# deepalcoholic/mlcomp

Measured on AMD Instinct MI355X. Metric: images/sec (whole node) ResNet-50 DAG train task, higher is better.
Workload: dtype bf16; 1 GPU; model=resnet50, global_batch=512, per_gpu_batch=512, image_size=224, parallelism=dp1, impl=native, optimizer=SGD momentum 0.9, wd 5e-5, fp32 master weights

## Files before the change

csrc/kernels/igemm.hip:

```cpp
#include "gfx950.h"
#include "convgeom.h"
#include <stdlib.h>
#include <map>
#include <mutex>
#include <vector>
#include <algorithm>
#include <cstdio>

namespace igemm {

constexpr int BK = 64, NTHR = 256;


template <int R>
__device__ __forceinline__ int mc_off(int k, int c) {
  if (R == 64) return k * 128 + ((c ^ (((k >> 1) & 1) << 2)) << 4);
  return k * (R * 2) + ((c ^ ((k & 3) << 2)) << 4);
}

template <class L, int R>
__device__ __forceinline__ void store_stage(char* lds, int tid, const uint4 (&v)[R / 32]) {
#pragma unroll
  for (int i = 0; i < R / 32; ++i) *reinterpret_cast<uint4*>(lds + L::lds_off(i, tid)) = v[i];
}
// ... 472 lines not shown
      ldg8f(bn.sc + st.ci[c], a);
      ldg8f(bn.sh + st.ci[c], b);
#pragma unroll
      for (int j = 0; j < 2; ++j) {
        const bool ok = (unsigned)(hb[j] + st.rd[c]) < (unsigned)g.H && (unsigned)(wb[j] + st.sd[c]) < (unsigned)g.W;
        v[2 * c + j] = bn_relu8(v[2 * c + j], a, b, ok);
      }
    }
  }
};


struct IdentityRows {
  __device__ __forceinline__ size_t operator()(int m) const { return (size_t)m; }
};
struct ClassRows {
  DgradClass c; int H, W;
  __device__ __forceinline__ size_t operator()(int m) const {
    int n, i, j;
    c.decode(m, n, i, j);
    return ((size_t)n * H + i * c.S + c.ph) * W + j * c.S + c.pw;
  }
};

struct BnBwdEpi {
  const bf16* mask = nullptr;
  const bf16* y0 = nullptr; const float* mean0 = nullptr; float* sums0 = nullptr;
  const bf16* y1 = nullptr; const float* mean1 = nullptr; float* sums1 = nullptr;
  const float* msc0 = nullptr; const float* msh0 = nullptr;
  const float* msc1 = nullptr; const float* msh1 = nullptr;
  int ncopy = NSTAT;
};

__device__ __forceinline__ float erf_from_exp(float x, float e) {
  const float t = __builtin_amdgcn_rcpf(1.f + 0.3275911f * fabsf(x));
  const float p = ((((1.061405429f * t - 1.453152027f) * t + 1.421413741f) * t - 0.284496736f) * t + 0.254829592f) * t;
  return copysignf(1.f - p * e, x);
}

__device__ __forceinline__ void dense_act8(float (&a)[8], int act, bf16* pre) {
  const int mode = act & 3;
  if (mode == 3) {
    if (pre) *reinterpret_cast<uint4*>(pre) = pack8(a);
#pragma unroll
    for (int e = 0; e < 8; ++e) a[e] = fmaxf(a[e], 0.f);
    return;
// ... 105 lines not shown
      if (aff) { ldg8f(bn.msc0 + ncl, ma0); ldg8f(bn.msh0 + ncl, mb0); }
      if (aff1) { ldg8f(bn.msc1 + ncl, ma1); ldg8f(bn.msh1 + ncl, mb1); }
    }
    const bool dense = kDense && (bias || act || dact);
    float bz[8];
#pragma unroll
    for (int e = 0; e < 8; ++e) bz[e] = 0.f;
    if (kDense && bias) ldg8f(bias + (nc < N ? nc : 0), bz);
    constexpr int ITERS = (BM + RPI - 1) / RPI;
    if (!addend && !red && !dense) {
#pragma unroll
      for (int it = 0; it < ITERS; ++it) {
        const int row = tid / CPR + RPI * it;
        const int m = m0 + row;
        if ((EXACT || (tok && row < BM)) && m < M && nc < N)
          *reinterpret_cast<uint4*>(out + rowmap(m) * ld + nc) =
              *reinterpret_cast<const uint4*>(lds + row * RS + c * 16);
      }
      return;
    }
    constexpr int UMAX = kDense ? 4 : 8;
    constexpr int U = ITERS < UMAX ? ITERS : UMAX;
    const bool has_add = addend != nullptr, has_mask = red && bn.mask, has_y1 = red && bn.y1;
#pragma unroll 1
    for (int it0 = 0; it0 < ITERS; it0 += U) {
      constexpr int UB = kDense ? 1 : U;
      constexpr int UD = kDense ? U : 1;
      uint4 vv[U], aa[U], zz[UB], p0[UB], p1[UB], du[UD];
      size_t off[U];
      bool ok[U];
#pragma unroll
      for (int u = 0; u < U; ++u) {
        int row = tid / CPR + RPI * (it0 + u);
        const bool rin = EXACT || (tok && row < BM);
        if (!rin) row = 0;
        const int m = m0 + row;
        ok[u] = rin && m < M && nc < N;
        off[u] = ok[u] ? rowmap(m) * ld + nc : 0;
        vv[u] = *reinterpret_cast<const uint4*>(lds + row * RS + c * 16);
        const uint4 zero = make_uint4(0u, 0u, 0u, 0u);
        aa[u] = has_add ? ldg16(addend + off[u]) : zero;
        if constexpr (!kDense) {
          zz[u] = has_mask ? ldg16(bn.mask + off[u]) : zero;
          p0[u] = red ? ldg16(bn.y0 + off[u]) : zero;
          p1[u] = has_y1 ? ldg16(bn.y1 + off[u]) : zero;
        }
        if constexpr (kDense) du[u] = dact ? ldg16(dact + off[u]) : zero;
      }
#pragma unroll
      for (int u = 0; u < U; ++u) {
        if (!ok[u]) continue;
        uint4 v = vv[u];
        if (has_add || red || dense) {
          float a[8];
          unpack8(v, a);
          if constexpr (kDense) {
          if (bias) {
#pragma unroll
            for (int e = 0; e < 8; ++e) a[e] += bz[e];
          }
          dense_act8(a, act, preact ? preact + off[u] : nullptr);
          if (dact) dense_dact8(a, act, du[u]);
          }
          if (has_add) {
            float b[8];
            unpack8(aa[u], b);
#pragma unroll
            for (int e = 0; e < 8; ++e) a[e] += b[e];
          }
          if constexpr (!kDense) {
            if (has_mask) {
              float z[8];
              unpack8(zz[u], z);
#pragma unroll
              for (int e = 0; e < 8; ++e) a[e] = z[e] > 0.f ? a[e] : 0.f;
            } else if (aff) {
              float y[8], q[8];
              unpack8(p0[u], y);
#pragma unroll
              for (int e = 0; e < 8; ++e) q[e] = y[e] * ma0[e] + mb0[e];
              if (aff1) {
                unpack8(p1[u], y);
#pragma unroll
                for (int e = 0; e < 8; ++e) q[e] += y[e] * ma1[e] + mb1[e];
              }
#pragma unroll
              for (int e = 0; e < 8; ++e) a[e] = q[e] > 0.f ? a[e] : 0.f;
// ... 897 lines not shown
  const MkMatKC fb{w, K, Co, K};
  if (KH == 1 && KW == 1 && stride == 1 && pad == 0) {
    if (in_sc) return launch_tiles(tile, M, Co, K, 1, st, epi, MkMatKCBn{x, C, M, K, bn}, fb);
    return launch_tiles(tile, M, Co, K, 1, st, epi, MkMatKC{x, C, M, K}, fb);
  }
  const ConvGeom g = mkgeom(N, H, W, C, Co, KH, KW, stride, pad, dil, Ho, Wo);
  if (in_sc) return launch_tiles(tile, M, Co, K, 1, st, epi, MkConvFwdABn{x, g, M, K, bn}, fb);
  return launch_tiles(tile, M, Co, K, 1, st, epi, MkConvFwdA{x, g, M, K}, fb);
}

MLC_EXPORT int mlc_conv_fwd(const bf16* x, const bf16* w, bf16* y, float* sum, float* sumsq,
                            int N, int H, int W, int C, int Co, int KH, int KW, int stride,
                            int pad, int dil, int Ho, int Wo, const float* in_sc, const float* in_sh,
                            hipStream_t st) {
  return conv_fwd_impl(x, w, y, Co, sum, sumsq, N, H, W, C, Co, KH, KW, stride, pad, dil, Ho, Wo, in_sc, in_sh, st);
}

MLC_EXPORT int mlc_conv_fwd_ld(const bf16* x, const bf16* w, bf16* y, int ldy, int N, int H, int W, int C, int Co,
                               int KH, int KW, int stride, int pad, int dil, int Ho, int Wo, hipStream_t st) {
  return conv_fwd_impl(x, w, y, ldy, nullptr, nullptr, N, H, W, C, Co, KH, KW, stride, pad, dil, Ho, Wo, nullptr,
                       nullptr, st);
}

static int dgrad_check(const BnBwdEpi& bn, int N, int H, int W, int C, int Co, int KH, int KW, int stride,
                       const float* sum, const float* sumsq) {
  if (C % 8 || Co % 8 || KH > 15 || KW > 16 || stride < 1 || ((sum == nullptr) != (sumsq == nullptr))) return -1;
  if (bn.y0 && g_mlc_det && ((long)N * H * W + 63) / 64 > g_mlc_ncopy) return -2;
  if (bn.msc0 && (!bn.msh0 || !bn.y0 || (bn.msc1 && (!bn.msh1 || !bn.y1)))) return -1;
  if (bn.y0 && (!bn.mean0 || !bn.sums0 || (bn.y1 && (!bn.mean1 || !bn.sums1)))) return -1;
  return 0;
}

template <class MkB>
static int dgrad_classes(const bf16* dy, const bf16* w, bf16* dx, const bf16* addend, const BnBwdEpi& bn,
                         const ConvGeom& g, int pad, float* sum, float* sumsq, hipStream_t st) {
  hipError_t err = hipSuccess;
  for (int ph = 0; ph < g.stride && ph < g.H; ++ph)
    for (int pw = 0; pw < g.stride && pw < g.W; ++pw) {
      const DgradClass cl = mkclass(g.stride, ph, pw, g.H, g.W, g.Ho, g.Wo, g.Co, g.KH, g.KW, pad, g.dil);
      if (cl.nr > 15 || cl.ns > 16) return -1;
      const int M = g.N * cl.Hc * cl.Wc, K = cl.nr * cl.ns * cl.ncb * BK;
      if (M <= 0) continue;
      if (sum && g_mlc_det && (M + 63) / 64 > g_mlc_ncopy) return -2;
      const int tile = pick_tile(M, g.C);
      const MkConvDgradA fa{dy, g, M, K, cl};
      const MkB fb{w, g, cl};
      if (g.stride == 1) {
        EpiBF16<> epi{dx, g.C, sum, sumsq, IdentityRows{}, addend, bn};
        epi.ncopy = g_mlc_ncopy;
        err = launch_tiles(tile, M, g.C, K, 1, st, epi, fa, fb);
      } else {
        EpiBF16<ClassRows> epi{dx, g.C, sum, sumsq, ClassRows{cl, g.H, g.W}, addend, bn};
        epi.ncopy = g_mlc_ncopy;
        err = launch_tiles(tile, M, g.C, K, 1, st, epi, fa, fb);
      }
      if (err != hipSuccess) return err;
    }
  return err;
}

static int conv_dgrad_impl(const bf16* dy, const bf16* w, bf16* dx, const bf16* addend, int N,
                           int H, int W, int C, int Co, int KH, int KW, int stride, int pad,
                           int dil, int Ho, int Wo, const bf16* bn_mask, const bf16* bn_y0,
                           const float* bn_mean0, float* bn_sums0, const bf16* bn_y1,
                           const float* bn_mean1, float* bn_sums1, const float* bn_msc0,
                           const float* bn_msh0, const float* bn_msc1, const float* bn_msh1,
                           float* sum, float* sumsq, hipStream_t st) {
  const BnBwdEpi bn{bn_mask, bn_y0, bn_mean0, bn_sums0, bn_y1, bn_mean1, bn_sums1,
                    bn_msc0, bn_msh0, bn_msc1, bn_msh1, g_mlc_ncopy};
  if (const int rc = dgrad_check(bn, N, H, W, C, Co, KH, KW, stride, sum, sumsq)) return rc;
  const ConvGeom g = mkgeom(N, H, W, C, Co, KH, KW, stride, pad, dil, Ho, Wo);
  if (KH == 1 && KW == 1 && stride == 1 && pad == 0) {
    const DgradClass cl = mkclass(1, 0, 0, H, W, Ho, Wo, Co, 1, 1, 0, dil);
    const int M = N * H * W, K = cl.ncb * BK;
    if (sum && g_mlc_det && (M + 63) / 64 > g_mlc_ncopy) return -2;
    EpiBF16<> epi{dx, C, sum, sumsq, IdentityRows{}, addend, bn};
    epi.ncopy = g_mlc_ncopy;
    return launch_tiles(pick_tile(M, C), M, C, K, 1, st, epi, MkMatKC{dy, Co, M, Co}, MkConvDgradB{w, g, cl});
  }
  return dgrad_classes<MkConvDgradB>(dy, w, dx, addend, bn, g, pad, sum, sumsq, st);
}

MLC_EXPORT int mlc_conv_dgrad(const bf16* dy, const bf16* w, bf16* dx, const bf16* addend, int N,
                              int H, int W, int C, int Co, int KH, int KW, int stride, int pad,
                              int dil, int Ho, int Wo, const bf16* bn_mask, const bf16* bn_y0,
                              const float* bn_mean0, float* bn_sums0, const bf16* bn_y1,
                              const float* bn_mean1, float* bn_sums1, const float* bn_msc0,
                              const float* bn_msh0, const float* bn_msc1, const float* bn_msh1,
                              hipStream_t st) {
  return conv_dgrad_impl(dy, w, dx, addend, N, H, W, C, Co, KH, KW, stride, pad, dil, Ho, Wo, bn_mask, bn_y0,
                         bn_mean0, bn_sums0, bn_y1, bn_mean1, bn_sums1, bn_msc0, bn_msh0, bn_msc1, bn_msh1,
                         nullptr, nullptr, st);
}

MLC_EXPORT int mlc_conv_tr_fwd(const bf16* x, const bf16* w, bf16* y, float* sum, float* sumsq, int N, int Hi,
                               int Wi, int Cin, int Cout, int KH, int KW, int stride, int pad, int dil, int Ho,
                               int Wo, hipStream_t st) {
  int pad_h, pad_w;
  unpack_pad(pad, pad_h, pad_w);
  if (Hi != (Ho + 2 * pad_h - dil * (KH - 1) - 1) / stride + 1 || Wi != (Wo + 2 * pad_w - dil * (KW - 1) - 1) / stride + 1)
    return -1;
  return conv_dgrad_impl(x, w, y, nullptr, N, Ho, Wo, Cout, Cin, KH, KW, stride, pad, dil, Hi, Wi, nullptr,
                         nullptr, nullptr, nullptr, nullptr, nullptr, nullptr, nullptr, nullptr, nullptr,
                         nullptr, sum, sumsq, st);
}

MLC_EXPORT int mlc_conv_dgrad_t(const bf16* dy, const bf16* wt, bf16* dx, const bf16* addend, int N,
                                int H, int W, int C, int Co, int KH, int KW, int stride, int pad,
                                int dil, int Ho, int Wo, const bf16* bn_mask, const bf16* bn_y0,
                                const float* bn_mean0, float* bn_sums0, const bf16* bn_y1,
                                const float* bn_mean1, float* bn_sums1, const float* bn_msc0,
                                const float* bn_msh0, const float* bn_msc1, const float* bn_msh1,
                                hipStream_t st) {
  const BnBwdEpi bn{bn_mask, bn_y0, bn_mean0, bn_sums0, bn_y1, bn_mean1, bn_sums1,
                    bn_msc0, bn_msh0, bn_msc1, bn_msh1, g_mlc_ncopy};
  if (const int rc = dgrad_check(bn, N, H, W, C, Co, KH, KW, stride, nullptr, nullptr)) return rc;
  int pad_h, pad_w;
  unpack_pad(pad, pad_h, pad_w);
  const int ph = dil * (KH - 1) - pad_h, pw = dil * (KW - 1) - pad_w;
  if (stride == 1 && ph >= 0 && pw >= 0) {
    if (Ho != H + 2 * pad_h - dil * (KH - 1) || Wo != W + 2 * pad_w - dil * (KW - 1)) return -1;
    const int M = N * H * W, K = KH * KW * Co;
    const int tile = pick_tile(M, C);
    EpiBF16<> epi{dx, C, nullptr, nullptr, IdentityRows{}, addend, bn};
    const MkMatKC fb{wt, K, C, K};
    if (KH == 1 && KW == 1) return launch_tiles(tile, M, C, K, 1, st, epi, MkMatKC{dy, Co, M, Co}, fb);
    const ConvGeom gf = mkgeom(N, Ho, Wo, Co, C, KH, KW, 1, pack_pad(ph, pw), dil, H, W);
    return launch_tiles(tile, M, C, K, 1, st, epi, MkConvFwdA{dy, gf, M, K}, fb);
  }
  const ConvGeom g = mkgeom(N, H, W, C, Co, KH, KW, stride, pad, dil, Ho, Wo);
  return dgrad_classes<MkConvDgradBT>(dy, wt, dx, addend, bn, g, pad, nullptr, nullptr, st);
}

namespace {
__global__ void __launch_bounds__(256)
splitk_reduce_kernel(const float* __restrict__ ws, float* __restrict__ out, long n4, int splits,
                     long slab4, int accumulate) {
  typedef float v4 __attribute__((ext_vector_type(4)));
  const v4* w4 = reinterpret_cast<const v4*>(ws);
  v4* o4 = reinterpret_cast<v4*>(out);
  for (long i = (long)blockIdx.x * 256 + threadIdx.x; i < n4; i += (long)gridDim.x * 256) {
    v4 a = accumulate ? o4[i] : (v4){0.f, 0.f, 0.f, 0.f};
    v4 b = {0.f, 0.f, 0.f, 0.f};
    int k = 0;
    for (; k + 4 <= splits; k += 4) {
      const v4 u0 = w4[(k + 0) * slab4 + i], u1 = w4[(k + 1) * slab4 + i];
      const v4 u2 = w4[(k + 2) * slab4 + i], u3 = w4[(k + 3) * slab4 + i];
      a += u0 + u1;
      b += u2 + u3;
    }
    for (; k < splits; ++k) a += w4[k * slab4 + i];
    o4[i] = a + b;
  }
}
// ... 237 lines not shown
```

mlcomp_amd/ops/_lib.py:

```python
from __future__ import annotations

import ctypes as C
import os
import threading

import torch

_LIB = None
_LOCK = threading.Lock()

DETERMINISTIC = os.environ.get('MLC_DETERMINISTIC', '0') == '1'
DET_COPIES = max(32, int(os.environ.get('MLC_DET_COPIES', '4096')))

vp, i32, i64, f32, u32 = C.c_void_p, C.c_int, C.c_long, C.c_float, C.c_uint

_SIGS = {
    'mlc_conv_fwd': [vp, vp, vp, vp, vp] + [i32] * 12 + [vp, vp, vp],
    'mlc_conv_fwd_ld': [vp, vp, vp] + [i32] * 13 + [vp],
    'mlc_conv_dgrad': [vp] * 4 + [i32] * 12 + [vp] * 11 + [vp],
    'mlc_conv_dgrad_t': [vp] * 4 + [i32] * 12 + [vp] * 11 + [vp],
    'mlc_bilinear_up_fwd': [vp, vp] + [i32] * 6 + [vp],
    'mlc_bilinear_up_bwd': [vp, vp] + [i32] * 6 + [vp],
    'mlc_gn_relu_fwd': [vp, vp, vp, vp, vp] + [i32] * 4 + [f32, vp],
    'mlc_gn_relu_bwd': [vp] * 7 + [i32] * 4 + [f32, vp],
    'mlc_conv_tr_fwd': [vp] * 5 + [i32] * 12 + [vp],
    'mlc_wt_transpose': [vp, i32, i64, vp],
    'mlc_conv_wgrad': [vp, vp, vp] + [i32] * 14 + [vp, i64, vp, vp, vp],
    'mlc_conv_wgrad_native': [vp, vp, vp] + [i32] * 14 + [vp, i64, vp, vp, vp],
    'mlc_gemm_f32out': [vp, vp, vp, vp] + [i32] * 11 + [vp],
    'mlc_gemm_bf16out': [vp, vp, vp] + [i32] * 8 + [vp],
    'mlc_gemm256_nt': [vp, vp, vp, vp] + [i32] * 6 + [vp, i32, vp, vp, i32, i32, vp],
    'mlc_g256_dense': [vp, vp, vp] + [i32] * 7 + [vp, i32, vp, vp, vp, i32, vp],
    'mlc_gemm256_tn': [vp, vp, vp] + [i32] * 8 + [vp],
    'mlc_conv256_fwd': [vp] * 5 + [i32] * 13 + [vp],
    'mlc_augment': [vp, vp, vp, vp] + [i32] * 7 + [vp],
    'mlc_augment_seg': [vp] * 6 + [i32] * 9 + [vp],
    'mlc_gemm_bf16_ex': [vp, vp, vp] + [i32] * 8 + [vp, i32, vp, vp, vp, vp, i64, vp],
    'mlc_gemm_bf16_ex_native': [vp, vp, vp] + [i32] * 8 + [vp, i32, vp, vp, vp, vp, i64, vp],
    'mlc_ln_fwd': [vp] * 8 + [i32, i32, f32, f32, f32, vp, u32, u32, vp],
    'mlc_ln_bwd': [vp] * 10 + [i32, i32, f32, f32, vp, u32, u32, vp],
    'mlc_ln_finalize_many': [vp, i32, i32, vp],
    'mlc_embed_bwd': [vp] * 7 + [i32] * 4 + [vp],
    'mlc_softmax_fwd': [vp] * 4 + [i64, i32, i32, f32, f32, vp, u32, vp],
# ... 175 lines not shown
```

mlcomp_amd/ops/functional.py:

```python
from __future__ import annotations

from typing import Optional, Tuple

import contextlib
import math
import os
import threading

import torch
import torch.nn.functional as F

from . import _lib


def _cuda(t):
    return t is not None and t.is_cuda


def conv_out_hw(H, W, KH, KW, stride, pad, dil):
    ph, pw = (pad, pad) if isinstance(pad, int) else tuple(pad)
    Ho = (H + 2 * ph - dil * (KH - 1) - 1) // stride + 1
    Wo = (W + 2 * pw - dil * (KW - 1) - 1) // stride + 1
    return Ho, Wo

# ... 191 lines not shown
        rows, blk = [], 0
        for s, v in zip(self.slots, self.views):
            Co, KH, KW, Ci = self._dims(s.shape)
            rows.append([s.bf16.data_ptr(), v.data_ptr(), Co, KH * KW, Ci, blk])
            blk += KH * KW * ((Co + 63) // 64) * ((Ci + 63) // 64)
        self.desc = torch.tensor(rows, dtype=torch.int64).to(self.buf.device)
        self.blocks = blk
        self._srcs = [r[0] for r in rows]

    def refresh(self):
        if self.buf is None:
            return
        if not self.buf.is_cuda:
            for s, v in zip(self.slots, self.views):
                v.copy_(wt_flip_transpose(s.bf16) if s.bf16.dim() == 4 else s.bf16.t())
            return
        if self._srcs != [s.bf16.data_ptr() for s in self.slots]:
            self._build()
        _lib.call('mlc_wt_transpose', _lib.ptr(self.desc), len(self.slots), self.blocks, _lib.stream())


def conv2d_dgrad(dy: torch.Tensor, w: torch.Tensor, x_shape, stride=1, pad=0, dil=1,
                 addend: Optional[torch.Tensor] = None, out: Optional[torch.Tensor] = None,
                 bn: Optional[BnBwdSpec] = None, wt: Optional[torch.Tensor] = None) -> torch.Tensor:
    N, H, W, C = x_shape
    Co, KH, KW, Ci = w.shape
    _, Ho, Wo, _ = dy.shape
    if _cuda(dy):
        dx = out if out is not None else torch.empty(N, H, W, C, device=dy.device, dtype=torch.bfloat16)
        b = [None] * 11
        if bn is not None:
            b[0] = bn.mask
            for k, (yk, mk, sk) in enumerate(bn.ys):
                b[1 + 3 * k:4 + 3 * k] = [yk, mk, sk]
            for k, (ak, hk) in enumerate(bn.affine or []):
                b[7 + 2 * k:9 + 2 * k] = [ak, hk]
        if wt is not None:
            assert tuple(wt.shape) == (Ci, KH, KW, Co), (wt.shape, w.shape)
            _lib.call('mlc_conv_dgrad_t', _lib.ptr(dy), _lib.ptr(wt), _lib.ptr(dx), _lib.ptr(addend), N, H, W,
                      C, Co, KH, KW, stride, pack_pad(pad), dil, Ho, Wo, *[_lib.ptr(t) for t in b], _lib.stream())
            return dx
        _lib.call('mlc_conv_dgrad', _lib.ptr(dy), _lib.ptr(w), _lib.ptr(dx), _lib.ptr(addend), N, H, W, C,
                  Co, KH, KW, stride, pack_pad(pad), dil, Ho, Wo, *[_lib.ptr(t) for t in b], _lib.stream())
        return dx
    if wt is not None and isinstance(pad, int) and dgrad_as_fwd_conv(KH, KW, stride, pad, dil):
        dxf = F.conv2d(dy.permute(0, 3, 1, 2).float(), wt.permute(0, 3, 1, 2).float(), None, 1,
                       dil * (KH - 1) - pad, dil)
    else:
        if wt is not None:
            w = wt_flip_transpose(wt)
        dxf = torch.nn.grad.conv2d_input((N, C, H, W), w.permute(0, 3, 1, 2).float(),
                                         dy.permute(0, 3, 1, 2).float(), stride, pad, dil)
    dxf = dxf.permute(0, 2, 3, 1)
    if addend is not None:
        dxf = dxf + addend.float()
    if bn is not None:
        if bn.mask is not None:
            dxf = dxf * (bn.mask.float() > 0)
        elif bn.affine is not None:
            q = sum(yk.float() * ak + hk for (yk, _, _), (ak, hk) in zip(bn.ys, bn.affine))
            dxf = dxf * (q > 0)
        d = dxf.to(torch.bfloat16).float().reshape(-1, C)
        for yk, mk, sk in bn.ys:
            sv = sk.view(NSTAT, 2, C)
            sv[0, 0] += d.sum(0)
            sv[0, 1] += (d * (yk.float().reshape(-1, C) - mk)).sum(0)
    dx = dxf.to(torch.bfloat16).contiguous()
    if out is not None:
        out.copy_(dx)
        return out
    return dx


_USE_SLAB = os.environ.get('MLC_WGRAD_SLAB', '1') != '0'
_SLAB = {}
_SLAB_OLD = []


# ... 1200 lines not shown
```

mlcomp_amd/ops/layers.py:

```python
from __future__ import annotations

import math
import os
from typing import List, Optional

import torch
import torch.nn as nn

from . import functional as Fn
from .arena import ParamArena, Slot

DGRAD_FIRST_ENV = os.environ.get('MLC_DGRAD_FIRST')


class Workspace:

    def __init__(self):
        self._req: List[tuple] = []
        self.buf = None
        self.views = {}

    def request(self, key, n):
        self._req.append((key, int(n)))
        return key

    def finalize(self, device):
        total = sum((n + 63) // 64 * 64 for _, n in self._req) or 64
        self.buf = torch.zeros(total, device=device, dtype=torch.float32)
        off = 0
        for key, n in self._req:
            self.views[key] = self.buf[off:off + n]
            off += (n + 63) // 64 * 64

    def __getitem__(self, key):
        return self.views[key]
# ... 221 lines not shown
        if self.s2d and in_affine is None:
            return Fn.stem_conv_fwd(x, self.w.bf16, stats=stats)
        if stats is not None and in_affine is None and self._conv1x1_fwd_ok(x):
            return Fn.conv1x1_fwd(x, self.w.bf16, stats)
        return Fn.conv2d_fwd(x, self.w.bf16, self.stride, self.pad, self.dil, stats=stats, in_affine=in_affine)

    def _conv1x1_fwd_ok(self, x) -> bool:
        if not (Fn.CONV1X1_FWD and x.is_cuda and type(self) is ConvBN and not self.s2d):
            return False
        if self.k != (1, 1) or self.stride != 1 or self.pad != 0 or x.shape[-1] != self.cin_p:
            return False
        return Fn.conv1x1_fwd_available(self.cin_p, self.Co)

    def _conv1x1_res_ok(self, x) -> bool:
        if not (Fn.CONV1X1_RES and x.is_cuda and type(self) is ConvBN and not self.s2d):
            return False
        if self.k != (1, 1) or self.stride != 1 or self.pad != 0 or x.shape[-1] != self.cin_p:
            return False
        min_rows = Fn.conv1x1_res_min_rows(self.cin_p, self.Co)
        if min_rows is None or math.prod(x.shape[:-1]) < min_rows:
            return False
        return Fn.conv1x1_fwd_res_available(self.cin_p, self.Co)

    def _dgrad(self, dy, x_shape, addend=None, out=None, bn=None):
        wt = None
        if self.wt_idx is not None:
            if self.ctx.wt_stale:
                raise RuntimeError('transposed filters are stale: the model must call '
                                   'ctx.refresh_wt() after its training forward pass')
            wt = self.ctx.wt[self.wt_idx]
        return Fn.conv2d_dgrad(dy, self.w.bf16, x_shape, self.stride, self.pad, self.dil,
                               addend=addend, out=out, bn=bn, wt=wt)

    def dgrad_covers_all(self) -> bool:
        return True

    def bn_target(self, rec):
        x, y, z = rec
        return (y, self.save_mean, self.ctx.ws[self.k_bw])

    def wgrad(self, dy, x, in_affine=None):
        Fn.conv2d_wgrad(dy, x, self.w.shape, self.stride, self.pad, self.dil, out=self.w.grad,
                        accumulate=self.ctx.grad_prezeroed, in_affine=in_affine, slab=self.ctx.wgrad_slab)
        if self.s2d:
            self.w.grad.mul_(self._gmask)

    def _fused_1x1_bwd_ok(self, dz, x, dgrad_bn) -> bool:
        if not (Fn.FUSE_1X1_BWD and dz.is_cuda and type(self) is ConvBN and not self.s2d):
            return False
        if self.k != (1, 1) or self.stride != 1 or self.pad != 0 or x.shape[-1] != self.cin_p:
            return False
        if dgrad_bn is not None and (dgrad_bn.mask is not None or len(dgrad_bn.ys) != 1
                                     or dgrad_bn.affine is None):
            return False
        return Fn.conv1x1_bn_bwd_available(self.cin_p, self.Co)

    def bwd(self, dz, rec, want_dres=False, dx_addend=None, need_dx=True, dx_out=None,
            prereduced=False, dgrad_bn=None, in_affine=None, defer: Optional[list] = None):
        x, y, z = rec
        arena = self.ctx.arena
        if need_dx and prereduced and in_affine is None and self._fused_1x1_bwd_ok(dz, x, dgrad_bn):
            if not self.ctx.grad_prezeroed:
                self.w.grad.zero_()
            dx = Fn.conv1x1_bn_bwd(dz, y, x, self.w.bf16, self.save_mean, self.save_invstd,
                                   self.gamma.master, self.ctx.ws[self.k_bw], self.gamma.grad,
                                   self.beta.grad, self.w.grad, addend=dx_addend, out=dx_out, bn=dgrad_bn)
            arena.mark_ready(self.gamma)
            arena.mark_ready(self.beta)
            arena.mark_ready(self.w)
            return dx, (dz if want_dres else None)
        dy, dres = Fn.bn_bwd(dz, z if self.act else None, y, self.save_mean, self.save_invstd,
                             self.gamma.master, want_dres=want_dres, dgamma=self.gamma.grad,
                             dbeta=self.beta.grad, sums=self.ctx.ws[self.k_bw], zero_sums=False,
                             coef=self.coef, prereduced=prereduced)
        arena.mark_ready(self.gamma)
        arena.mark_ready(self.beta)
        side = self.ctx.wgrad_stream if need_dx else None
        if side is not None and torch.cuda.current_stream(self.ctx.device) == side:
            side = None
        fork = None
        if side is not None:
            main = torch.cuda.current_stream(self.ctx.device)
            fork = torch.cuda.Event()
            fork.record(main)
            if not self.ctx.dgrad_first:
                side.wait_event(fork)
                with Fn.side_stream(side):
                    self.wgrad(dy, x, in_affine)
        else:
            self.wgrad(dy, x, in_affine)
        dx = None
        if need_dx:
            dx = self._dgrad(dy, x.shape, addend=dx_addend, out=dx_out, bn=dgrad_bn)
        if side is not None and self.ctx.dgrad_first:
            side.wait_event(fork)
            with Fn.side_stream(side):
                self.wgrad(dy, x, in_affine)
        if side is not None and defer is not None:
            defer.append((dy, x, self.w))
            return dx, dres
        if side is not None and self.ctx.wgrad_defer:
            dy.record_stream(side)
            x.record_stream(side)
            arena.mark_ready(self.w)
            return dx, dres
        if side is not None and self.ctx.wgrad_lag:
            ev = torch.cuda.Event()
            ev.record(side)
            self.ctx.lag_wgrad(ev, (dy, x), self.w)
            return dx, dres
        if side is not None:
            main.wait_stream(side)
        arena.mark_ready(self.w)
        return dx, dres


# ... 31 lines not shown
    def load_from_torch(self):
        super().load_from_torch()
        b = self._bias()
        if b is not None:
            self.run_mean.sub_(b)

    def export_to_torch(self):
        super().export_to_torch()
        b = self._bias()
        if b is not None:
            bn = self._src[1]
            bn.running_mean.add_(b.to(bn.running_mean.device))

    def out_hw(self, H, W):
        KH, KW = self.k
        return ((H - 1) * self.stride - 2 * self.pad + self.dil * (KH - 1) + self.out_pad[0] + 1,
                (W - 1) * self.stride - 2 * self.pad + self.dil * (KW - 1) + self.out_pad[1] + 1)

    def _conv(self, x, stats, in_affine=None):
        assert in_affine is None
        return Fn.conv_transpose2d_fwd(x, self.w.bf16, self.out_hw(x.shape[1], x.shape[2]), self.stride,
                                       self.pad, self.dil, stats=stats)

    def _dgrad(self, dy, x_shape, addend=None, out=None, bn=None):
        assert addend is None and out is None and bn is None, 'ConvTBN input gradient: plain conv'
        dx = Fn.conv2d_fwd(dy, self.w.bf16, self.stride, self.pad, self.dil)
        assert tuple(dx.shape) == tuple(x_shape), (dx.shape, x_shape)
        return dx

    def wgrad(self, dy, x, in_affine=None):
        assert in_affine is None
        Fn.conv2d_wgrad(x, dy, self.w.shape, self.stride, self.pad, self.dil, out=self.w.grad,
                        accumulate=self.ctx.grad_prezeroed)


class _ConvBNFn(torch.autograd.Function):
    @staticmethod
    def forward(ctx, x, res, anchor, m: ConvBN):
        z, rec = m.fwd(x, res)
        ctx.m = m
        ctx.has_res = res is not None
        ctx.save_for_backward(*rec)
        return z

    @staticmethod
    def backward(ctx, dz):
        m: ConvBN = ctx.m
        dx, dres = m.bwd(dz.contiguous(), ctx.saved_tensors, want_dres=ctx.has_res,
# ... 105 lines not shown
        blk.dout_prereduced = False
        units = blk.units
        fuse = blk.fuse_bn_bwd
        affs = blk.in_affines()
        if blk.fuse_bn_fwd:
            assert fuse, 'the BN-apply fusion needs the fused BN-backward reductions (z is not stored)'

        def spec_for(i):
            u = units[i]
            if not fuse or not units[i + 1].dgrad_covers_all():
                return None
            if u.act:
                return Fn.BnBwdSpec(None, [u.bn_target(recs[i])], affine=[(u.scale, u.shift)])
            return Fn.BnBwdSpec(None, [u.bn_target(recs[i])])

        side = units[0].ctx.wgrad_stream
        pend = [] if side is not None and os.environ.get('MLC_WGRAD_STREAM') == '2' else None
        sp = spec_for(len(units) - 2) if len(units) > 1 else None
        d, dres = units[-1].bwd(dout, recs[-1], want_dres=True, prereduced=pre, dgrad_bn=sp,
                                in_affine=affs[-1], defer=pend)
        fused = sp is not None
        down_side = side if (blk.down is not None and pend is None and blk.down_stream) else None
        short = dres
        if down_side is not None:
            main = torch.cuda.current_stream(units[0].ctx.device)
            short_buf = torch.empty(rd[0].shape, device=rd[0].device, dtype=rd[0].dtype) if need_dx else None
            down_side.wait_stream(main)
            with Fn.side_stream(down_side):
                short, _ = blk.down.bwd(dres, rd, need_dx=need_dx, prereduced=pre, dx_out=short_buf)
        for i in range(len(units) - 2, 0, -1):
            sp = spec_for(i - 1)
            d, _ = units[i].bwd(d, recs[i], prereduced=fused, dgrad_bn=sp, in_affine=affs[i], defer=pend)
            fused = sp is not None
        if down_side is not None:
            main.wait_stream(down_side)
        elif blk.down is not None:
            short, _ = blk.down.bwd(dres, rd, need_dx=need_dx, prereduced=pre, defer=pend)
        prev_spec = None
        if need_dx and fuse and blk.prev is not None and blk.prev._last is not None \
                and units[0].dgrad_covers_all():
            prev_spec = blk.prev.output_bn_spec()
        dx, _ = units[0].bwd(d, recs[0], dx_addend=short if need_dx else None, need_dx=need_dx,
                             dx_out=short if (need_dx and blk.down is not None) else None,
                             prereduced=fused, dgrad_bn=prev_spec, defer=pend)
        if prev_spec is not None:
            blk.prev.dout_prereduced = True
        if pend:
            torch.cuda.current_stream(units[0].ctx.device).wait_stream(side)
            for _, _, w in pend:
                units[0].ctx.arena.mark_ready(w)
            pend.clear()
        return dx, None, None


class MaxPool:
    def __init__(self, k=3, s=2, p=1):
        self.k, self.s, self.p = k, s, p

    def __call__(self, x, anchor):
        return _MaxPoolFn.apply(x, anchor, self)


class _MaxPoolFn(torch.autograd.Function):
    @staticmethod
    def forward(ctx, x, anchor, m):
        y, idx = Fn.maxpool_fwd(x, m.k, m.s, m.p)
        ctx.m = m
# ... 114 lines not shown
```

Before: 14420 images/s.

## Compute strided 1x1 shortcut dgrad compactly and scatter-add it in dgrad epilogue

For strided 1x1 downsample convs, the shortcut input gradient is now computed at the output resolution only, as a compact tensor, instead of a full-resolution dx that is mostly zeros. The block's first conv dgrad epilogue then adds this compact gradient at the strided positions, decoding each pixel with fast division. This removes the zero-filled work and memory traffic of the strided dgrad. In exchange it adds per-row divmod work in the epilogue, bypasses the fused 1x1 backward path whenever a strided addend is present, and allocates a new epilogue template instantiation.

Measured after the change: 14600 images/s, median of 6. +1.2%, better.

```diff
diff --git a/csrc/kernels/igemm.hip b/csrc/kernels/igemm.hip
--- a/csrc/kernels/igemm.hip
+++ b/csrc/kernels/igemm.hip
@@ -518,6 +518,22 @@
     return ((size_t)n * H + i * c.S + c.ph) * W + j * c.S + c.pw;
   }
 };
+template <class Rows = IdentityRows>
+struct StridedAddRows {
+  Rows rows; int Ho, Wo; FastDiv fW, fH, fS;
+  __device__ __forceinline__ size_t operator()(int m) const { return rows(m); }
+  __device__ __forceinline__ bool addend_pixel(size_t pix, size_t& cpix) const {
+    unsigned t, n, h, w, hq, hr, wq, wr;
+    fW.divmod((unsigned)pix, t, w);
+    fH.divmod(t, n, h);
+    fS.divmod(h, hq, hr);
+    fS.divmod(w, wq, wr);
+    cpix = ((size_t)n * Ho + hq) * Wo + wq;
+    return (hr | wr) == 0;
+  }
+};
+template <class R> struct HasStridedAdd { static constexpr bool value = false; };
+template <class R> struct HasStridedAdd<StridedAddRows<R>> { static constexpr bool value = true; };
 
 struct BnBwdEpi {
   const bf16* mask = nullptr;
@@ -669,13 +685,14 @@
     constexpr int UMAX = kDense ? 4 : 8;
     constexpr int U = ITERS < UMAX ? ITERS : UMAX;
     const bool has_add = addend != nullptr, has_mask = red && bn.mask, has_y1 = red && bn.y1;
+    constexpr bool kSAdd = HasStridedAdd<RowMap>::value;
 #pragma unroll 1
     for (int it0 = 0; it0 < ITERS; it0 += U) {
       constexpr int UB = kDense ? 1 : U;
       constexpr int UD = kDense ? U : 1;
       uint4 vv[U], aa[U], zz[UB], p0[UB], p1[UB], du[UD];
       size_t off[U];
-      bool ok[U];
+      bool ok[U], hit[U];
 #pragma unroll
       for (int u = 0; u < U; ++u) {
         int row = tid / CPR + RPI * (it0 + u);
@@ -683,10 +700,18 @@
         if (!rin) row = 0;
         const int m = m0 + row;
         ok[u] = rin && m < M && nc < N;
-        off[u] = ok[u] ? rowmap(m) * ld + nc : 0;
+        const size_t pix = ok[u] ? rowmap(m) : 0;
+        off[u] = ok[u] ? pix * ld + nc : 0;
         vv[u] = *reinterpret_cast<const uint4*>(lds + row * RS + c * 16);
         const uint4 zero = make_uint4(0u, 0u, 0u, 0u);
-        aa[u] = has_add ? ldg16(addend + off[u]) : zero;
+        if constexpr (kSAdd) {
+          size_t cpix = 0;
+          hit[u] = has_add && ok[u] && rowmap.addend_pixel(pix, cpix);
+          aa[u] = hit[u] ? ldg16(addend + cpix * ld + nc) : zero;
+        } else {
+          hit[u] = has_add;
+          aa[u] = has_add ? ldg16(addend + off[u]) : zero;
+        }
         if constexpr (!kDense) {
           zz[u] = has_mask ? ldg16(bn.mask + off[u]) : zero;
           p0[u] = red ? ldg16(bn.y0 + off[u]) : zero;
@@ -709,7 +734,7 @@
           dense_act8(a, act, preact ? preact + off[u] : nullptr);
           if (dact) dense_dact8(a, act, du[u]);
           }
-          if (has_add) {
+          if (hit[u]) {
             float b[8];
             unpack8(aa[u], b);
 #pragma unroll
@@ -1653,17 +1678,39 @@
                        nullptr, st);
 }
 
-static int dgrad_check(const BnBwdEpi& bn, int N, int H, int W, int C, int Co, int KH, int KW, int stride,
-                       const float* sum, const float* sumsq) {
+struct DgradAddend {
+  const bf16* same = nullptr; const bf16* compact = nullptr; int S = 1;
+};
+
+static int dgrad_check(const BnBwdEpi& bn, const DgradAddend& add, int N, int H, int W, int C, int Co, int KH,
+                       int KW, int stride, const float* sum, const float* sumsq) {
   if (C % 8 || Co % 8 || KH > 15 || KW > 16 || stride < 1 || ((sum == nullptr) != (sumsq == nullptr))) return -1;
+  if (add.S < 1 || (add.compact && add.same)) return -1;
   if (bn.y0 && g_mlc_det && ((long)N * H * W + 63) / 64 > g_mlc_ncopy) return -2;
   if (bn.msc0 && (!bn.msh0 || !bn.y0 || (bn.msc1 && (!bn.msh1 || !bn.y1)))) return -1;
   if (bn.y0 && (!bn.mean0 || !bn.sums0 || (bn.y1 && (!bn.mean1 || !bn.sums1)))) return -1;
   return 0;
 }
 
+template <class Rows, class FA, class FB>
+static hipError_t launch_dgrad(const Rows& rows, bf16* dx, const DgradAddend& add, const BnBwdEpi& bn, float* sum,
+                               float* sumsq, int H, int W, int M, int C, int K, hipStream_t st, const FA& fa,
+                               const FB& fb) {
+  const int tile = pick_tile(M, C);
+  if (add.compact) {
+    const StridedAddRows<Rows> srows{rows, (H - 1) / add.S + 1, (W - 1) / add.S + 1, FastDiv(W), FastDiv(H),
+                                     FastDiv(add.S)};
+    EpiBF16<StridedAddRows<Rows>> epi{dx, C, sum, sumsq, srows, add.compact, bn};
+    epi.ncopy = g_mlc_ncopy;
+    return launch_tiles(tile, M, C, K, 1, st, epi, fa, fb);
+  }
+  EpiBF16<Rows> epi{dx, C, sum, sumsq, rows, add.same, bn};
+  epi.ncopy = g_mlc_ncopy;
+  return launch_tiles(tile, M, C, K, 1, st, epi, fa, fb);
+}
+
 template <class MkB>
-static int dgrad_classes(const bf16* dy, const bf16* w, bf16* dx, const bf16* addend, const BnBwdEpi& bn,
+static int dgrad_classes(const bf16* dy, const bf16* w, bf16* dx, const DgradAddend& add, const BnBwdEpi& bn,
                          const ConvGeom& g, int pad, float* sum, float* sumsq, hipStream_t st) {
   hipError_t err = hipSuccess;
   for (int ph = 0; ph < g.stride && ph < g.H; ++ph)
@@ -1673,24 +1720,18 @@
       const int M = g.N * cl.Hc * cl.Wc, K = cl.nr * cl.ns * cl.ncb * BK;
       if (M <= 0) continue;
       if (sum && g_mlc_det && (M + 63) / 64 > g_mlc_ncopy) return -2;
-      const int tile = pick_tile(M, g.C);
       const MkConvDgradA fa{dy, g, M, K, cl};
       const MkB fb{w, g, cl};
-      if (g.stride == 1) {
-        EpiBF16<> epi{dx, g.C, sum, sumsq, IdentityRows{}, addend, bn};
-        epi.ncopy = g_mlc_ncopy;
-        err = launch_tiles(tile, M, g.C, K, 1, st, epi, fa, fb);
-      } else {
-        EpiBF16<ClassRows> epi{dx, g.C, sum, sumsq, ClassRows{cl, g.H, g.W}, addend, bn};
-        epi.ncopy = g_mlc_ncopy;
-        err = launch_tiles(tile, M, g.C, K, 1, st, epi, fa, fb);
-      }
+      if (g.stride == 1)
+        err = launch_dgrad(IdentityRows{}, dx, add, bn, sum, sumsq, g.H, g.W, M, g.C, K, st, fa, fb);
+      else
+        err = launch_dgrad(ClassRows{cl, g.H, g.W}, dx, add, bn, sum, sumsq, g.H, g.W, M, g.C, K, st, fa, fb);
       if (err != hipSuccess) return err;
     }
   return err;
 }
 
-static int conv_dgrad_impl(const bf16* dy, const bf16* w, bf16* dx, const bf16* addend, int N,
+static int conv_dgrad_impl(const bf16* dy, const bf16* w, bf16* dx, const DgradAddend& add, int N,
                            int H, int W, int C, int Co, int KH, int KW, int stride, int pad,
                            int dil, int Ho, int Wo, const bf16* bn_mask, const bf16* bn_y0,
                            const float* bn_mean0, float* bn_sums0, const bf16* bn_y1,
@@ -1699,17 +1740,16 @@
                            float* sum, float* sumsq, hipStream_t st) {
   const BnBwdEpi bn{bn_mask, bn_y0, bn_mean0, bn_sums0, bn_y1, bn_mean1, bn_sums1,
                     bn_msc0, bn_msh0, bn_msc1, bn_msh1, g_mlc_ncopy};
-  if (const int rc = dgrad_check(bn, N, H, W, C, Co, KH, KW, stride, sum, sumsq)) return rc;
+  if (const int rc = dgrad_check(bn, add, N, H, W, C, Co, KH, KW, stride, sum, sumsq)) return rc;
   const ConvGeom g = mkgeom(N, H, W, C, Co, KH, KW, stride, pad, dil, Ho, Wo);
   if (KH == 1 && KW == 1 && stride == 1 && pad == 0) {
     const DgradClass cl = mkclass(1, 0, 0, H, W, Ho, Wo, Co, 1, 1, 0, dil);
     const int M = N * H * W, K = cl.ncb * BK;
     if (sum && g_mlc_det && (M + 63) / 64 > g_mlc_ncopy) return -2;
-    EpiBF16<> epi{dx, C, sum, sumsq, IdentityRows{}, addend, bn};
-    epi.ncopy = g_mlc_ncopy;
-    return launch_tiles(pick_tile(M, C), M, C, K, 1, st, epi, MkMatKC{dy, Co, M, Co}, MkConvDgradB{w, g, cl});
-  }
-  return dgrad_classes<MkConvDgradB>(dy, w, dx, addend, bn, g, pad, sum, sumsq, st);
+    return launch_dgrad(IdentityRows{}, dx, add, bn, sum, sumsq, H, W, M, C, K, st, MkMatKC{dy, Co, M, Co},
+                        MkConvDgradB{w, g, cl});
+  }
+  return dgrad_classes<MkConvDgradB>(dy, w, dx, add, bn, g, pad, sum, sumsq, st);
 }
 
 MLC_EXPORT int mlc_conv_dgrad(const bf16* dy, const bf16* w, bf16* dx, const bf16* addend, int N,
@@ -1719,9 +1759,21 @@
                               const float* bn_mean1, float* bn_sums1, const float* bn_msc0,
                               const float* bn_msh0, const float* bn_msc1, const float* bn_msh1,
                               hipStream_t st) {
-  return conv_dgrad_impl(dy, w, dx, addend, N, H, W, C, Co, KH, KW, stride, pad, dil, Ho, Wo, bn_mask, bn_y0,
-                         bn_mean0, bn_sums0, bn_y1, bn_mean1, bn_sums1, bn_msc0, bn_msh0, bn_msc1, bn_msh1,
+  return conv_dgrad_impl(dy, w, dx, DgradAddend{addend}, N, H, W, C, Co, KH, KW, stride, pad, dil, Ho, Wo, bn_mask,
+                         bn_y0, bn_mean0, bn_sums0, bn_y1, bn_mean1, bn_sums1, bn_msc0, bn_msh0, bn_msc1, bn_msh1,
                          nullptr, nullptr, st);
+}
+
+MLC_EXPORT int mlc_conv_dgrad_sadd(const bf16* dy, const bf16* w, bf16* dx, const bf16* addend, const bf16* sadd,
+                                   int sadd_stride, int N, int H, int W, int C, int Co, int KH, int KW,
+                                   int stride, int pad, int dil, int Ho, int Wo, const bf16* bn_mask,
+                                   const bf16* bn_y0, const float* bn_mean0, float* bn_sums0, const bf16* bn_y1,
+                                   const float* bn_mean1, float* bn_sums1, const float* bn_msc0,
+                                   const float* bn_msh0, const float* bn_msc1, const float* bn_msh1,
+                                   hipStream_t st) {
+  return conv_dgrad_impl(dy, w, dx, DgradAddend{addend, sadd, sadd_stride}, N, H, W, C, Co, KH, KW, stride, pad, dil,
+                         Ho, Wo, bn_mask, bn_y0, bn_mean0, bn_sums0, bn_y1, bn_mean1, bn_sums1, bn_msc0, bn_msh0,
+                         bn_msc1, bn_msh1, nullptr, nullptr, st);
 }
 
 MLC_EXPORT int mlc_conv_tr_fwd(const bf16* x, const bf16* w, bf16* y, float* sum, float* sumsq, int N, int Hi,
@@ -1731,9 +1783,37 @@
   unpack_pad(pad, pad_h, pad_w);
   if (Hi != (Ho + 2 * pad_h - dil * (KH - 1) - 1) / stride + 1 || Wi != (Wo + 2 * pad_w - dil * (KW - 1) - 1) / stride + 1)
     return -1;
-  return conv_dgrad_impl(x, w, y, nullptr, N, Ho, Wo, Cout, Cin, KH, KW, stride, pad, dil, Hi, Wi, nullptr,
+  return conv_dgrad_impl(x, w, y, DgradAddend{}, N, Ho, Wo, Cout, Cin, KH, KW, stride, pad, dil, Hi, Wi, nullptr,
                          nullptr, nullptr, nullptr, nullptr, nullptr, nullptr, nullptr, nullptr, nullptr,
                          nullptr, sum, sumsq, st);
+}
+
+static int conv_dgrad_t_impl(const bf16* dy, const bf16* wt, bf16* dx, const DgradAddend& add, int N,
+                             int H, int W, int C, int Co, int KH, int KW, int stride, int pad,
+                             int dil, int Ho, int Wo, const bf16* bn_mask, const bf16* bn_y0,
+                             const float* bn_mean0, float* bn_sums0, const bf16* bn_y1,
+                             const float* bn_mean1, float* bn_sums1, const float* bn_msc0,
+                             const float* bn_msh0, const float* bn_msc1, const float* bn_msh1,
+                             hipStream_t st) {
+  const BnBwdEpi bn{bn_mask, bn_y0, bn_mean0, bn_sums0, bn_y1, bn_mean1, bn_sums1,
+                    bn_msc0, bn_msh0, bn_msc1, bn_msh1, g_mlc_ncopy};
+  if (const int rc = dgrad_check(bn, add, N, H, W, C, Co, KH, KW, stride, nullptr, nullptr)) return rc;
+  int pad_h, pad_w;
+  unpack_pad(pad, pad_h, pad_w);
+  const int ph = dil * (KH - 1) - pad_h, pw = dil * (KW - 1) - pad_w;
+  if (stride == 1 && ph >= 0 && pw >= 0) {
+    if (Ho != H + 2 * pad_h - dil * (KH - 1) || Wo != W + 2 * pad_w - dil * (KW - 1)) return -1;
+    const int M = N * H * W, K = KH * KW * Co;
+    const MkMatKC fb{wt, K, C, K};
+    if (KH == 1 && KW == 1)
+      return launch_dgrad(IdentityRows{}, dx, add, bn, nullptr, nullptr, H, W, M, C, K, st, MkMatKC{dy, Co, M, Co},
+                          fb);
+    const ConvGeom gf = mkgeom(N, Ho, Wo, Co, C, KH, KW, 1, pack_pad(ph, pw), dil, H, W);
+    return launch_dgrad(IdentityRows{}, dx, add, bn, nullptr, nullptr, H, W, M, C, K, st, MkConvFwdA{dy, gf, M, K},
+                        fb);
+  }
+  const ConvGeom g = mkgeom(N, H, W, C, Co, KH, KW, stride, pad, dil, Ho, Wo);
+  return dgrad_classes<MkConvDgradBT>(dy, wt, dx, add, bn, g, pad, nullptr, nullptr, st);
 }
 
 MLC_EXPORT int mlc_conv_dgrad_t(const bf16* dy, const bf16* wt, bf16* dx, const bf16* addend, int N,
@@ -1743,24 +1823,21 @@
                                 const float* bn_mean1, float* bn_sums1, const float* bn_msc0,
                                 const float* bn_msh0, const float* bn_msc1, const float* bn_msh1,
                                 hipStream_t st) {
-  const BnBwdEpi bn{bn_mask, bn_y0, bn_mean0, bn_sums0, bn_y1, bn_mean1, bn_sums1,
-                    bn_msc0, bn_msh0, bn_msc1, bn_msh1, g_mlc_ncopy};
-  if (const int rc = dgrad_check(bn, N, H, W, C, Co, KH, KW, stride, nullptr, nullptr)) return rc;
-  int pad_h, pad_w;
-  unpack_pad(pad, pad_h, pad_w);
-  const int ph = dil * (KH - 1) - pad_h, pw = dil * (KW - 1) - pad_w;
-  if (stride == 1 && ph >= 0 && pw >= 0) {
-    if (Ho != H + 2 * pad_h - dil * (KH - 1) || Wo != W + 2 * pad_w - dil * (KW - 1)) return -1;
-    const int M = N * H * W, K = KH * KW * Co;
-    const int tile = pick_tile(M, C);
-    EpiBF16<> epi{dx, C, nullptr, nullptr, IdentityRows{}, addend, bn};
-    const MkMatKC fb{wt, K, C, K};
-    if (KH == 1 && KW == 1) return launch_tiles(tile, M, C, K, 1, st, epi, MkMatKC{dy, Co, M, Co}, fb);
-    const ConvGeom gf = mkgeom(N, Ho, Wo, Co, C, KH, KW, 1, pack_pad(ph, pw), dil, H, W);
-    return launch_tiles(tile, M, C, K, 1, st, epi, MkConvFwdA{dy, gf, M, K}, fb);
-  }
-  const ConvGeom g = mkgeom(N, H, W, C, Co, KH, KW, stride, pad, dil, Ho, Wo);
-  return dgrad_classes<MkConvDgradBT>(dy, wt, dx, addend, bn, g, pad, nullptr, nullptr, st);
+  return conv_dgrad_t_impl(dy, wt, dx, DgradAddend{addend}, N, H, W, C, Co, KH, KW, stride, pad, dil, Ho, Wo,
+                           bn_mask, bn_y0, bn_mean0, bn_sums0, bn_y1, bn_mean1, bn_sums1, bn_msc0, bn_msh0, bn_msc1,
+                           bn_msh1, st);
+}
+
+MLC_EXPORT int mlc_conv_dgrad_t_sadd(const bf16* dy, const bf16* wt, bf16* dx, const bf16* addend, const bf16* sadd,
+                                     int sadd_stride, int N, int H, int W, int C, int Co, int KH, int KW,
+                                     int stride, int pad, int dil, int Ho, int Wo, const bf16* bn_mask,
+                                     const bf16* bn_y0, const float* bn_mean0, float* bn_sums0, const bf16* bn_y1,
+                                     const float* bn_mean1, float* bn_sums1, const float* bn_msc0,
+                                     const float* bn_msh0, const float* bn_msc1, const float* bn_msh1,
+                                     hipStream_t st) {
+  return conv_dgrad_t_impl(dy, wt, dx, DgradAddend{addend, sadd, sadd_stride}, N, H, W, C, Co, KH, KW, stride, pad,
+                           dil, Ho, Wo, bn_mask, bn_y0, bn_mean0, bn_sums0, bn_y1, bn_mean1, bn_sums1, bn_msc0,
+                           bn_msh0, bn_msc1, bn_msh1, st);
 }
 
 namespace {
diff --git a/mlcomp_amd/ops/_lib.py b/mlcomp_amd/ops/_lib.py
--- a/mlcomp_amd/ops/_lib.py
+++ b/mlcomp_amd/ops/_lib.py
@@ -19,6 +19,8 @@
     'mlc_conv_fwd_ld': [vp, vp, vp] + [i32] * 13 + [vp],
     'mlc_conv_dgrad': [vp] * 4 + [i32] * 12 + [vp] * 11 + [vp],
     'mlc_conv_dgrad_t': [vp] * 4 + [i32] * 12 + [vp] * 11 + [vp],
+    'mlc_conv_dgrad_sadd': [vp] * 5 + [i32] * 13 + [vp] * 11 + [vp],
+    'mlc_conv_dgrad_t_sadd': [vp] * 5 + [i32] * 13 + [vp] * 11 + [vp],
     'mlc_bilinear_up_fwd': [vp, vp] + [i32] * 6 + [vp],
     'mlc_bilinear_up_bwd': [vp, vp] + [i32] * 6 + [vp],
     'mlc_gn_relu_fwd': [vp, vp, vp, vp, vp] + [i32] * 4 + [f32, vp],
diff --git a/mlcomp_amd/ops/functional.py b/mlcomp_amd/ops/functional.py
--- a/mlcomp_amd/ops/functional.py
+++ b/mlcomp_amd/ops/functional.py
@@ -237,10 +237,16 @@
 
 def conv2d_dgrad(dy: torch.Tensor, w: torch.Tensor, x_shape, stride=1, pad=0, dil=1,
                  addend: Optional[torch.Tensor] = None, out: Optional[torch.Tensor] = None,
-                 bn: Optional[BnBwdSpec] = None, wt: Optional[torch.Tensor] = None) -> torch.Tensor:
+                 bn: Optional[BnBwdSpec] = None, wt: Optional[torch.Tensor] = None,
+                 strided_addend: Optional[Tuple[torch.Tensor, int]] = None) -> torch.Tensor:
     N, H, W, C = x_shape
     Co, KH, KW, Ci = w.shape
     _, Ho, Wo, _ = dy.shape
+    if strided_addend is not None:
+        assert addend is None, 'one addend form at a time'
+        sadd, S = strided_addend
+        assert S >= 1 and tuple(sadd.shape) == (N, (H - 1) // S + 1, (W - 1) // S + 1, C), (sadd.shape, x_shape, S)
+        assert sadd.is_contiguous() and (out is None or out.data_ptr() != sadd.data_ptr())
     if _cuda(dy):
         dx = out if out is not None else torch.empty(N, H, W, C, device=dy.device, dtype=torch.bfloat16)
         b = [None] * 11
@@ -250,13 +256,15 @@
                 b[1 + 3 * k:4 + 3 * k] = [yk, mk, sk]
             for k, (ak, hk) in enumerate(bn.affine or []):
                 b[7 + 2 * k:9 + 2 * k] = [ak, hk]
+        name, filt = 'mlc_conv_dgrad', w
         if wt is not None:
             assert tuple(wt.shape) == (Ci, KH, KW, Co), (wt.shape, w.shape)
-            _lib.call('mlc_conv_dgrad_t', _lib.ptr(dy), _lib.ptr(wt), _lib.ptr(dx), _lib.ptr(addend), N, H, W,
-                      C, Co, KH, KW, stride, pack_pad(pad), dil, Ho, Wo, *[_lib.ptr(t) for t in b], _lib.stream())
-            return dx
-        _lib.call('mlc_conv_dgrad', _lib.ptr(dy), _lib.ptr(w), _lib.ptr(dx), _lib.ptr(addend), N, H, W, C,
-                  Co, KH, KW, stride, pack_pad(pad), dil, Ho, Wo, *[_lib.ptr(t) for t in b], _lib.stream())
+            name, filt = 'mlc_conv_dgrad_t', wt
+        add = [_lib.ptr(addend)]
+        if strided_addend is not None:
+            name, add = name + '_sadd', [None, _lib.ptr(sadd), S]
+        _lib.call(name, _lib.ptr(dy), _lib.ptr(filt), _lib.ptr(dx), *add, N, H, W, C, Co, KH, KW, stride,
+                  pack_pad(pad), dil, Ho, Wo, *[_lib.ptr(t) for t in b], _lib.stream())
         return dx
     if wt is not None and isinstance(pad, int) and dgrad_as_fwd_conv(KH, KW, stride, pad, dil):
         dxf = F.conv2d(dy.permute(0, 3, 1, 2).float(), wt.permute(0, 3, 1, 2).float(), None, 1,
@@ -269,6 +277,9 @@
     dxf = dxf.permute(0, 2, 3, 1)
     if addend is not None:
         dxf = dxf + addend.float()
+    if strided_addend is not None:
+        dxf = dxf.contiguous()
+        dxf[:, ::S, ::S, :] += sadd.float()
     if bn is not None:
         if bn.mask is not None:
             dxf = dxf * (bn.mask.float() > 0)
diff --git a/mlcomp_amd/ops/layers.py b/mlcomp_amd/ops/layers.py
--- a/mlcomp_amd/ops/layers.py
+++ b/mlcomp_amd/ops/layers.py
@@ -11,6 +11,7 @@
 from .arena import ParamArena, Slot
 
 DGRAD_FIRST_ENV = os.environ.get('MLC_DGRAD_FIRST')
+COMPACT_SHORTCUT_GRAD = os.environ.get('MLC_COMPACT_SHORTCUT_GRAD', '1') == '1'
 
 
 class Workspace:
@@ -278,15 +279,22 @@
             return False
         return Fn.conv1x1_fwd_res_available(self.cin_p, self.Co)
 
-    def _dgrad(self, dy, x_shape, addend=None, out=None, bn=None):
+    def _dgrad(self, dy, x_shape, addend=None, out=None, bn=None, saddend=None, compact=False):
         wt = None
         if self.wt_idx is not None:
             if self.ctx.wt_stale:
                 raise RuntimeError('transposed filters are stale: the model must call '
                                    'ctx.refresh_wt() after its training forward pass')
             wt = self.ctx.wt[self.wt_idx]
+        if compact:
+            assert self.compact_dx() and addend is None and saddend is None and bn is None
+            return Fn.conv2d_dgrad(dy, self.w.bf16, tuple(dy.shape[:3]) + (x_shape[3],), out=out, wt=wt)
         return Fn.conv2d_dgrad(dy, self.w.bf16, x_shape, self.stride, self.pad, self.dil,
-                               addend=addend, out=out, bn=bn, wt=wt)
+                               addend=addend, out=out, bn=bn, wt=wt, strided_addend=saddend)
+
+    def compact_dx(self) -> bool:
+        return (COMPACT_SHORTCUT_GRAD and type(self) is ConvBN and not self.s2d and self.k == (1, 1)
+                and self.pad == 0 and self.dil == 1 and self.stride > 1)
 
     def dgrad_covers_all(self) -> bool:
         return True
@@ -312,10 +320,12 @@
         return Fn.conv1x1_bn_bwd_available(self.cin_p, self.Co)
 
     def bwd(self, dz, rec, want_dres=False, dx_addend=None, need_dx=True, dx_out=None,
-            prereduced=False, dgrad_bn=None, in_affine=None, defer: Optional[list] = None):
+            prereduced=False, dgrad_bn=None, in_affine=None, defer: Optional[list] = None,
+            dx_saddend=None, compact_dx=False):
         x, y, z = rec
         arena = self.ctx.arena
-        if need_dx and prereduced and in_affine is None and self._fused_1x1_bwd_ok(dz, x, dgrad_bn):
+        if need_dx and prereduced and in_affine is None and dx_saddend is None \
+                and self._fused_1x1_bwd_ok(dz, x, dgrad_bn):
             if not self.ctx.grad_prezeroed:
                 self.w.grad.zero_()
             dx = Fn.conv1x1_bn_bwd(dz, y, x, self.w.bf16, self.save_mean, self.save_invstd,
@@ -347,7 +357,8 @@
             self.wgrad(dy, x, in_affine)
         dx = None
         if need_dx:
-            dx = self._dgrad(dy, x.shape, addend=dx_addend, out=dx_out, bn=dgrad_bn)
+            dx = self._dgrad(dy, x.shape, addend=dx_addend, out=dx_out, bn=dgrad_bn, saddend=dx_saddend,
+                             compact=compact_dx)
         if side is not None and self.ctx.dgrad_first:
             side.wait_event(fork)
             with Fn.side_stream(side):
@@ -425,8 +436,9 @@
         return Fn.conv_transpose2d_fwd(x, self.w.bf16, self.out_hw(x.shape[1], x.shape[2]), self.stride,
                                        self.pad, self.dil, stats=stats)
 
-    def _dgrad(self, dy, x_shape, addend=None, out=None, bn=None):
-        assert addend is None and out is None and bn is None, 'ConvTBN input gradient: plain conv'
+    def _dgrad(self, dy, x_shape, addend=None, out=None, bn=None, saddend=None, compact=False):
+        assert addend is None and out is None and bn is None and saddend is None and not compact, \
+            'ConvTBN input gradient: plain conv'
         dx = Fn.conv2d_fwd(dy, self.w.bf16, self.stride, self.pad, self.dil)
         assert tuple(dx.shape) == tuple(x_shape), (dx.shape, x_shape)
         return dx
@@ -578,12 +590,15 @@
         fused = sp is not None
         down_side = side if (blk.down is not None and pend is None and blk.down_stream) else None
         short = dres
+        compact = need_dx and blk.down is not None and blk.down.compact_dx()
         if down_side is not None:
             main = torch.cuda.current_stream(units[0].ctx.device)
-            short_buf = torch.empty(rd[0].shape, device=rd[0].device, dtype=rd[0].dtype) if need_dx else None
+            short_shape = tuple(dres.shape[:3]) + (rd[0].shape[3],) if compact else rd[0].shape
+            short_buf = torch.empty(short_shape, device=rd[0].device, dtype=rd[0].dtype) if need_dx else None
             down_side.wait_stream(main)
             with Fn.side_stream(down_side):
-                short, _ = blk.down.bwd(dres, rd, need_dx=need_dx, prereduced=pre, dx_out=short_buf)
+                short, _ = blk.down.bwd(dres, rd, need_dx=need_dx, prereduced=pre, dx_out=short_buf,
+                                        compact_dx=compact)
         for i in range(len(units) - 2, 0, -1):
             sp = spec_for(i - 1)
             d, _ = units[i].bwd(d, recs[i], prereduced=fused, dgrad_bn=sp, in_affine=affs[i], defer=pend)
@@ -591,14 +606,18 @@
         if down_side is not None:
             main.wait_stream(down_side)
         elif blk.down is not None:
-            short, _ = blk.down.bwd(dres, rd, need_dx=need_dx, prereduced=pre, defer=pend)
+            short, _ = blk.down.bwd(dres, rd, need_dx=need_dx, prereduced=pre, defer=pend, compact_dx=compact)
         prev_spec = None
         if need_dx and fuse and blk.prev is not None and blk.prev._last is not None \
                 and units[0].dgrad_covers_all():
             prev_spec = blk.prev.output_bn_spec()
-        dx, _ = units[0].bwd(d, recs[0], dx_addend=short if need_dx else None, need_dx=need_dx,
-                             dx_out=short if (need_dx and blk.down is not None) else None,
-                             prereduced=fused, dgrad_bn=prev_spec, defer=pend)
+        if compact:
+            dx, _ = units[0].bwd(d, recs[0], dx_saddend=(short, blk.down.stride), need_dx=need_dx,
+                                 prereduced=fused, dgrad_bn=prev_spec, defer=pend)
+        else:
+            dx, _ = units[0].bwd(d, recs[0], dx_addend=short if need_dx else None, need_dx=need_dx,
+                                 dx_out=short if (need_dx and blk.down is not None) else None,
+                                 prereduced=fused, dgrad_bn=prev_spec, defer=pend)
         if prev_spec is not None:
             blk.prev.dout_prereduced = True
         if pend:
```
